# RobinChen121/Stochastic-Inventory

Measured on NVIDIA B200. Metric: state-action-demand evaluations/s (fp64), full-horizon SDP solve, higher is better.
Workload: dtype f64

## Files before the change

stochastic-inventory_b200/csrc/kernel_lead.cuh:

```cuda
#pragma once
#include <cuda_runtime.h>

#include <cstdlib>

#include "dev_model.cuh"
#include "kernel_tiled.cuh"

namespace sdpb {

constexpr int kLeadYT = 4;

struct LeadArgs {
    int t, D, pmf_off;
    const double* Vn;
    double* Vt;
    int* Qt;
    long long lo, hi;
    long long row0;
    int NYT;
    int ny_tiles, nq2_tiles;
    int A, Apad, di_max, NR;
    int nthreads;
};

__device__ __forceinline__ long long lds_s64(unsigned shared_addr) {
    long long v;
    asm volatile("ld.shared.s64 %0, [%1];" : "=l"(v) : "r"(shared_addr));
    return v;
}

__device__ __forceinline__ double ldg_at(const char* base, long long byte_off) {
    return __ldg(reinterpret_cast<const double*>(base + byte_off));
}

__device__ __forceinline__ double lds_double(unsigned shared_addr) {
    double v;
    asm volatile("ld.shared.f64 %0, [%1];" : "=d"(v) : "r"(shared_addr));
    return v;
}

template <bool IS_MIN, bool LAST, int RQ, bool DEDUP>
__global__ void __launch_bounds__(256)
bi_lead_slab(const __grid_constant__ DevModel M, const __grid_constant__ LeadArgs a) {
    constexpr int YT = kLeadYT;
    extern __shared__ __align__(16) unsigned char smem_raw[];
    const int NYB = YT * a.NYT;
    const int D = a.D, A = a.A, Apad = a.Apad;
    double* slab = reinterpret_cast<double*>(smem_raw);
    const size_t slab_elems = (size_t)max(a.NR, NYB) * RQ * Apad;
    double* Lw = slab + slab_elems;
    double2* PP = reinterpret_cast<double2*>(Lw + ((a.NR + 1) & ~1));

    long long b = blockIdx.x;
    int q2_0 = 0;
    if (M.lead == 2) { q2_0 = (int)(b % a.nq2_tiles) * RQ; b /= a.nq2_tiles; }
    const int ytile = (int)(b % a.ny_tiles); b /= a.ny_tiles;
    const long long ix = DEDUP ? 0 : a.row0 + b;
    const int q1_0 = ytile * NYB;
    const long long y0 = ix + q1_0;
    const int n_levels = DEDUP ? (M.nI + M.nQ - 1) : M.nQ;

    const int tid = threadIdx.x;
    for (int j = tid; j < D; j += a.nthreads) PP[j] = make_double2(M.pmf_p[a.pmf_off + j], M.pmf_pg[a.pmf_off + j]);
    const bool lost = (M.flags & SDPB_F_LOST_SALES) != 0;
    const long long strideX = (M.lead == 2) ? (long long)M.nQ * M.nQ : (long long)M.nQ;
    for (int wi = tid; wi < a.NR; wi += a.nthreads) {
        const double lvl = M.inv_min + (double)(y0 - a.di_max + wi) * M.step;
        Lw[wi] = M.h * fmax(lvl, 0.0) + M.pen * fmax(-lvl, 0.0);
    }
    if (!LAST) {
        const int warp_s = tid >> 5, lane_s = tid & 31, nwarps_s = a.nthreads >> 5;
        for (int row = warp_s; row < a.NR * RQ; row += nwarps_s) {
            const int wi = row / RQ, rr = row - wi * RQ;
            long long is = y0 - a.di_max + wi;
            if (lost) is = is > M.i_zero ? is : M.i_zero;
            is = is < M.nI - 1 ? is : M.nI - 1;
            is = is > 0 ? is : 0;
            const int q2 = min(q2_0 + rr, M.nQ - 1);
            const double* __restrict__ src = a.Vn + is * strideX + ((M.lead == 2) ? (long long)q2 * M.nQ : 0);
            const unsigned dst = (unsigned)__cvta_generic_to_shared(slab + (size_t)row * Apad);
            for (int ai = lane_s; ai < A; ai += 32)
                asm volatile("cp.async.ca.shared.global [%0], [%1], 8;" ::"r"(dst + (unsigned)ai * 8u), "l"(src + ai));
        }
        asm volatile("cp.async.commit_group;");
        asm volatile("cp.async.wait_group 0;" ::: "memory");
    }
    __syncthreads();

    const int g = tid / A, ai = tid - g * A;
    const bool worker = g < a.NYT;
    double acc[YT][RQ];
#pragma unroll
    for (int k = 0; k < YT; k++)
#pragma unroll
        for (int r = 0; r < RQ; r++) acc[k][r] = 0.0;

    if (worker) {
        const double av = (double)ai * M.step;
        const double fv = (av > 0.0 ? M.K : 0.0) + M.v_t[a.t - 1] * av;
        const unsigned slab_s = (unsigned)__cvta_generic_to_shared(slab) + (unsigned)ai * 8u;
        const unsigned lw_s = (unsigned)__cvta_generic_to_shared(Lw);
        const unsigned pp_s = (unsigned)__cvta_generic_to_shared(PP);
        const unsigned row_bytes = (unsigned)(RQ * Apad) * 8u;
        int wi0 = YT * g + (D - 1);
        double cst[YT], Vw[YT][RQ];
#pragma unroll
        for (int k = 0; k < YT; k++) {
            cst[k] = fv + lds_double(lw_s + (unsigned)(wi0 + k) * 8u);
#pragma unroll
            for (int r = 0; r < RQ; r++)
                Vw[k][r] = LAST ? 0.0 : lds_double(slab_s + (unsigned)(wi0 + k) * row_bytes + (unsigned)(r * Apad) * 8u);
        }
#define SDPB_LEAD_STEP(JJ)                                                                          \
        {                                                                                               \
            const double2 pp = lds_double2(pp_s + (unsigned)j * 16u);                                   \
            const int wn = max(wi0 - 1, 0);                                                             \
            const double lnew = lds_double(lw_s + (unsigned)wn * 8u);                                   \
            double vnew[RQ];                                                                            \
            _Pragma("unroll") for (int r = 0; r < RQ; r++)                                              \
                vnew[r] = LAST ? 0.0 : lds_double(slab_s + (unsigned)wn * row_bytes + (unsigned)(r * Apad) * 8u); \
            _Pragma("unroll") for (int k = 0; k < YT; k++) {                                            \
                const int ph = (k - (JJ)) & 3;                                                          \
                const double m = pp.x * cst[ph];                                \
                _Pragma("unroll") for (int r = 0; r < RQ; r++) {                                        \
                    acc[k][r] += m;                                     \
                    if (!LAST) acc[k][r] += pp.y * Vw[ph][r];           \
                }                                                                                       \
            }                                                                                           \
            const int pn = (3 - (JJ)) & 3;                                                              \
            cst[pn] = fv + lnew;                                                                        \
            _Pragma("unroll") for (int r = 0; r < RQ; r++) Vw[pn][r] = vnew[r];                         \
            wi0 -= 1;                                                                                   \
            j += 1;                                                                                     \
        }
        int j = 0;
        for (; j + 4 <= D;) { SDPB_LEAD_STEP(0) SDPB_LEAD_STEP(1) SDPB_LEAD_STEP(2) SDPB_LEAD_STEP(3) }
        if (j < D) SDPB_LEAD_STEP(0)
        if (j < D) SDPB_LEAD_STEP(1)
        if (j < D) SDPB_LEAD_STEP(2)
#undef SDPB_LEAD_STEP
    }

    __syncthreads();
    double* Qs = slab;
    if (worker) {
#pragma unroll
        for (int k = 0; k < YT; k++)
#pragma unroll
            for (int r = 0; r < RQ; r++) Qs[((size_t)(YT * g + k) * RQ + r) * Apad + ai] = acc[k][r];
    }
    __syncthreads();
    const int warp = tid >> 5, lane = tid & 31, nwarps = a.nthreads >> 5;
    for (int s = warp; s < NYB * RQ; s += nwarps) {
        const int local = s / RQ, r = s - local * RQ;
        const double* q = Qs + (size_t)s * Apad;
        double best = IS_MIN ? DBL_MAX : -DBL_MAX;
        int besti = kNoAction;
        for (int i = lane; i < A; i += 32) {
            const double v = q[i];
            if (IS_MIN ? (v < best) : (v > best)) { best = v; besti = i; }
        }
#pragma unroll
        for (int sh = 16; sh > 0; sh >>= 1) {
            const double ov = __shfl_xor_sync(0xffffffffu, best, sh);
            const int oi = __shfl_xor_sync(0xffffffffu, besti, sh);
            if (better<IS_MIN>(ov, oi, best, besti)) { best = ov; besti = oi; }
        }
        if (lane == 0) {
            const int lev = q1_0 + local;
            const int q2 = q2_0 + r;
            if (lev < n_levels && (M.lead != 2 || q2 < M.nQ)) {
                long long idx = DEDUP ? (long long)lev : ix * M.nQ + lev;
                if (M.lead == 2) idx = idx * M.nQ + q2;
                if (idx >= a.lo && idx < a.hi) {
                    a.Vt[idx] = best;
                    a.Qt[idx] = besti == kNoAction ? -1 : besti;
                }
            }
        }
    }
}

struct LeadPlan {
    bool ok = false;
    int NYT = 0, RQ = 1, Apad = 0, nthreads = 0, di_max = 0, span = 0, NR = 0;
// ... 147 lines not shown
            double pre = 0.0;
            if (!LAST) pre = ldg_at(col, lds_s64(ro_s + (unsigned)max(wi0 - 1, 0) * 8u));
#define SDPB_COL_STEP(JJ)                                                                             \
            {                                                                                             \
                const double2 pp = lds_double2(pp_s + (unsigned)j * 16u);                                 \
                const double vnew = pre;                                                                  \
                if (!LAST) pre = ldg_at(col, lds_s64(ro_s + (unsigned)max(wi0 - 2, 0) * 8u));             \
                const double lnew = lds_double(lw_s + (unsigned)max(wi0 - 1, 0) * 8u);                    \
                _Pragma("unroll") for (int k = 0; k < YT; k++) {                                          \
                    const int ph = (k - (JJ)) & (YT - 1);                                                 \
                    acc[k] += pp.x * cst[ph];                             \
                    if (!LAST) acc[k] += pp.y * Vw[ph];                   \
                }                                                                                         \
                const int pn = (YT - 1 - (JJ)) & (YT - 1);                                                \
                cst[pn] = fv + lnew;                                                                      \
                Vw[pn] = vnew;                                                                            \
                wi0 -= 1;                                                                                 \
                j += 1;                                                                                   \
            }
            int j = 0;
            for (; j + YT <= D;) {
#pragma unroll
                for (int jj = 0; jj < YT; jj++) SDPB_COL_STEP(jj)
            }
#pragma unroll
            for (int jj = 0; jj < YT - 1; jj++)
                if (j < D) SDPB_COL_STEP(jj)
#undef SDPB_COL_STEP
        }
#pragma unroll
        for (int k = 0; k < YT; k++) red_v[(size_t)k * a.nthreads + tid] = acc[k];
        __syncthreads();
        for (int s = warp; s < YT * a.NQB; s += nwarps) {
            const int k = s / a.NQB, sq = s - k * a.NQB;
            const double* q = red_v + (size_t)k * a.nthreads + sq * A;
            double best = IS_MIN ? DBL_MAX : -DBL_MAX;
            int besti = kNoAction;
            for (int i = lane; i < A; i += 32) {
                const double v = q[i];
                if (IS_MIN ? (v < best) : (v > best)) { best = v; besti = i; }
            }
#pragma unroll
            for (int sh = 16; sh > 0; sh >>= 1) {
                const double ov = __shfl_xor_sync(0xffffffffu, best, sh);
                const int oi = __shfl_xor_sync(0xffffffffu, besti, sh);
                if (better<IS_MIN>(ov, oi, best, besti)) { best = ov; besti = oi; }
            }
            if (lane == 0) {
                const int lev = l0 + k;
                const int sq2 = q2g * a.NQB + sq;
                if (lev < l_end && (M.lead != 2 || sq2 < M.nQ)) {
                    long long idx = DEDUP ? (long long)lev : ix * M.nQ + lev;
                    if (M.lead == 2) idx = idx * M.nQ + sq2;
                    if (idx >= a.lo && idx < a.hi) {
                        a.Vt[idx] = best;
                        a.Qt[idx] = besti == kNoAction ? -1 : besti;
                    }
                }
            }
        }
    }
}

struct ColPlan {
    bool ok = false;
    int NQB = 1, nthreads = 0, LT = 0, di_max = 0, span = 0, NRW = 0;
    size_t smem = 0;
};

inline ColPlan plan_col(const sdpb_model& m, const DevModel& d, int D, const int* di, bool dedup) {
    ColPlan P;
    if (m.cost_kind != SDPB_COST_BACKORDER || m.lead_time < 1) return P;
    int lo = di[0], hi = di[0];
    for (int j = 0; j < D; j++) {
        if (di[j] != di[0] + j) return P;
        lo = std::min(lo, di[j]);
        hi = std::max(hi, di[j]);
    }
    const int A = d.max_order_idx + 1;
    if (A > 512) return P;
    const int max_threads = 512;
    P.NQB = m.lead_time == 2 ? std::max(1, std::min(max_threads / A, d.nQ)) : 1;
    P.nthreads = ((P.NQB * A + 31) / 32) * 32;
    const int n_levels = dedup ? d.nI + d.nQ - 1 : d.nQ;
    P.LT = dedup ? 64 : ((n_levels + kColYT - 1) / kColYT) * kColYT;
    P.di_max = hi;
    P.span = hi - lo;
    P.NRW = P.LT + P.span;
    P.smem = ((((size_t)2 * kColYT * P.nthreads + 2 * (size_t)P.NRW) * 8 + 15) & ~(size_t)15) + (size_t)D * 16 + 16;
    P.ok = P.smem <= 100 * 1024;
    return P;
}

template <bool DEDUP>
inline int launch_col(const ColPlan& P, const DevModel& dm, int t, int D, int pmf_off, const double* Vn,
                      double* Vt, int* Qt, long long lo, long long hi, cudaStream_t stream) {
    if (hi <= lo) return SDPB_OK;
    ColArgs a;
    a.t = t; a.D = D; a.pmf_off = pmf_off; a.Vn = Vn; a.Vt = Vt; a.Qt = Qt; a.lo = lo; a.hi = hi;
    a.A = dm.max_order_idx + 1; a.NQB = P.NQB; a.LT = P.LT; a.di_max = P.di_max; a.NRW = P.NRW;
    a.nthreads = P.nthreads;
    a.nq2_groups = dm.lead == 2 ? (dm.nQ + P.NQB - 1) / P.NQB : 1;
    const int n_levels = DEDUP ? dm.nI + dm.nQ - 1 : dm.nQ;
    a.n_ltiles = (n_levels + P.LT - 1) / P.LT;
    long long rows = 1;
    a.row0 = 0;
    if (!DEDUP) {
        const long long per_x = dm.lead == 2 ? (long long)dm.nQ * dm.nQ : (long long)dm.nQ;
        a.row0 = lo / per_x;
        rows = (hi - 1) / per_x - a.row0 + 1;
    }
    const long long blocks = rows * a.n_ltiles * a.nq2_groups;
    const bool last = (Vn == nullptr), mn = dm.is_min != 0;
    cudaError_t e = cudaSuccess;
#define SDPB_COL_LAUNCH(MN, LS)                                                                        \
    {                                                                                                  \
        auto k = bi_lead_col<MN, LS, DEDUP>;                                                           \
        if (P.smem > 48 * 1024) e = cudaFuncSetAttribute(k, cudaFuncAttributeMaxDynamicSharedMemorySize, (int)P.smem); \
        if (e == cudaSuccess) k<<<(unsigned)blocks, P.nthreads, P.smem, stream>>>(dm, a);              \
    }
    if (mn) { if (last) SDPB_COL_LAUNCH(true, true) else SDPB_COL_LAUNCH(true, false) }
    else    { if (last) SDPB_COL_LAUNCH(false, true) else SDPB_COL_LAUNCH(false, false) }
#undef SDPB_COL_LAUNCH
    if (e != cudaSuccess || cudaGetLastError() != cudaSuccess) return SDPB_ERR_CUDA;
    return SDPB_OK;
}

struct DevPeer { char* base0; unsigned long long stride; long long lo, hi; };

template <bool IS_MIN>
__global__ void __launch_bounds__(256)
merge_action_slices(const double* __restrict__ sv, const int* __restrict__ sa, int parts, long long n_local,
                    double* __restrict__ Vt, int* __restrict__ Qt, long long lo, const DevPeer* __restrict__ peers,
                    int n_peers, int t) {
    const long long i = (long long)blockIdx.x * blockDim.x + threadIdx.x;
    if (i >= n_local) return;
    double best = IS_MIN ? DBL_MAX : -DBL_MAX;
    int arg = kNoAction;
    for (int q = 0; q < parts; q++) {
        const double v = sv[(long long)q * n_local + i];
        const int av = sa[(long long)q * n_local + i];
        if (av != kNoAction && (IS_MIN ? (v < best) : (v > best))) { best = v; arg = av; }
    }
    Vt[i] = best;
    Qt[i] = arg == kNoAction ? -1 : arg;
    const long long idx = lo + i;
    for (int p = 0; p < n_peers; p++) {
        const DevPeer pr = peers[p];
        if (idx >= pr.lo && idx < pr.hi)
            reinterpret_cast<double*>(pr.base0 + (unsigned long long)(t - 1) * pr.stride)[idx] = best;
    }
}

struct Q2Args {
    int t, D, pmf_off;
    const double* VnT;
    double* Vt;
    int* Qt;
    long long lo, hi;
    long long f_begin, f_end;
    int n_chunks, tpx;
    int cs;
    double* slice_v;
    int* slice_a;
    int di_max, NRW;
    int parts;
    int n_peer;
    double* peer_v[2];
    long long peer_lo[2], peer_hi[2];
};

struct PeerStore { double* v; long long lo, hi; };

constexpr int kQ2YT = 8, kQ2PF = 2, kQ2PAD = kQ2PF + 1;

__global__ void transpose_q2a(const double* __restrict__ V, double* __restrict__ VT, int nQ, int row0) {
    __shared__ double tile[32][33];
    const long long base = (long long)(row0 + blockIdx.x) * nQ * nQ;
    const int c0 = blockIdx.y * 32, r0 = blockIdx.z * 32;
    for (int r = threadIdx.y; r < 32; r += 8) {
        const int row = r0 + r, c = c0 + threadIdx.x;
        if (row < nQ && c < nQ) tile[r][threadIdx.x] = V[base + (long long)row * nQ + c];
    }
    __syncthreads();
    for (int r = threadIdx.y; r < 32; r += 8) {
        const int row = c0 + r, c = r0 + threadIdx.x;
        if (row < nQ && c < nQ) VT[base + (long long)row * nQ + c] = tile[threadIdx.x][r];
    }
}

template <bool IS_MIN, bool LAST, int NT, int PARTS>
__global__ void __launch_bounds__(NT, 512 / NT)
bi_lead_q2(const __grid_constant__ DevModel M, const __grid_constant__ Q2Args a) {
    constexpr int YT = kQ2YT, PF = kQ2PF, W = YT + PF, PAD = kQ2PAD;
    extern __shared__ __align__(16) unsigned char smem_raw[];
    double2* WR = reinterpret_cast<double2*>(smem_raw);
    double2* PP = WR + a.NRW;
    const int D = a.D, nQ = M.nQ, tid = threadIdx.x;
    constexpr int cols = NT / PARTS;
    const int part = tid / cols, col = tid - part * cols;
    double* MV = reinterpret_cast<double*>(PP + D);
    int* MA = reinterpret_cast<int*>(MV + (size_t)(PARTS - 1) * YT * cols);
    const long long F0 = a.f_begin + (long long)blockIdx.x * cols;
    const long long x_first = F0 / a.tpx;
    const bool lost = (M.flags & SDPB_F_LOST_SALES) != 0;

    for (int j = tid; j < D; j += NT) PP[j] = make_double2(M.pmf_p[a.pmf_off + j], M.pmf_pg[a.pmf_off + j]);
    for (int wi = tid; wi < a.NRW; wi += NT) {
        const long long il = x_first - a.di_max - PAD + wi;
        const double lvl = M.inv_min + (double)il * M.step;
        long long is = il;
        if (lost) is = is > M.i_zero ? is : M.i_zero;
        is = is < M.nI - 1 ? is : M.nI - 1;
        is = is > 0 ? is : 0;
        WR[wi] = make_double2(M.h * fmax(lvl, 0.0) + M.pen * fmax(-lvl, 0.0),
                              __hiloint2double(0, (int)(is * nQ * nQ)));
    }
    __syncthreads();

    const long long F = min(F0 + col, a.f_end - 1);
    const long long x = F / a.tpx;
    const int f = (int)(F - x * a.tpx);
    const int chunk = f / nQ, q2 = f - chunk * nQ, l0 = chunk * YT;
    const long long idx0 = (x * nQ + l0) * nQ + q2;
    bool any = false;
#pragma unroll
    for (int k = 0; k < YT; k++) any |= (l0 + k < nQ) && idx0 + (long long)k * nQ >= a.lo && idx0 + (long long)k * nQ < a.hi;
    any = any && F0 + col < a.f_end;
    if (PARTS == 1 && !any) return;

    const unsigned wr0 = (unsigned)__cvta_generic_to_shared(WR) + (unsigned)((int)(x - x_first) + l0 + (D - 1) + PAD) * 16u;
    const unsigned pp_s = (unsigned)__cvta_generic_to_shared(PP);
    const double* __restrict__ cb = LAST ? nullptr : a.VnT + q2;
    const double vt = M.v_t[a.t - 1];

    double best[YT];
    int arg[YT];
#pragma unroll
    for (int k = 0; k < YT; k++) { best[k] = IS_MIN ? DBL_MAX : -DBL_MAX; arg[k] = kNoAction; }

    const int per_part = (M.max_order_idx + PARTS) / PARTS;
    const int ai_begin = any ? part * per_part : 0;
    const int ai_end = any ? min(M.max_order_idx + 1, ai_begin + per_part) : 0;
    if (!LAST) cb += (long long)ai_begin * nQ;
    for (int ai = ai_begin; ai < ai_end; ai++) {
        const double av = (double)ai * M.step;
        const double fv = (av > 0.0 ? M.K : 0.0) + vt * av;
        double acc[YT], cst[W], Vw[W];
#pragma unroll
        for (int k = 0; k < YT; k++) acc[k] = 0.0;
#pragma unroll
        for (int k = 0; k < W; k++) {
            const double2 e = lds_double2(wr0 + (unsigned)((k < YT ? k : k - W) * 16));
            cst[k] = fv + e.x;
            Vw[k] = LAST ? 0.0 : __ldg(cb + __double2loint(e.y));
        }
        unsigned wr_run = wr0 - (unsigned)((PF + 1) * 16);
#define SDPB_Q2_STEP(JJ)                                                                              \
        {                                                                                                 \
            const double2 pp = lds_double2(pp_s + (unsigned)j * 16u);                                     \
            _Pragma("unroll") for (int k = 0; k < YT; k++) {                                              \
                acc[k] += pp.x * cst[(k - (JJ) + W) % W];                 \
                if (!LAST) acc[k] += pp.y * Vw[(k - (JJ) + W) % W];       \
            }                                                                                             \
            const double2 e = lds_double2(wr_run);             \
            cst[(YT - 1 - (JJ) + W) % W] = fv + e.x;                                                      \
            if (!LAST) Vw[(YT - 1 - (JJ) + W) % W] = __ldg(cb + __double2loint(e.y));                     \
            wr_run -= 16u;                                                                                \
            j += 1;                                                                                       \
        }
        int j = 0;
        while (j + W <= D) {
#pragma unroll
            for (int JJ = 0; JJ < W; JJ++) SDPB_Q2_STEP(JJ)
        }
#pragma unroll
        for (int JJ = 0; JJ < W - 1; JJ++)
            if (j < D) SDPB_Q2_STEP(JJ)
#undef SDPB_Q2_STEP
#pragma unroll
        for (int k = 0; k < YT; k++)
            if (IS_MIN ? (acc[k] < best[k]) : (acc[k] > best[k])) { best[k] = acc[k]; arg[k] = ai; }
        if (!LAST) cb += nQ;
    }
    if (PARTS > 1) {
        if (part > 0) {
#pragma unroll
            for (int k = 0; k < YT; k++) {
                MV[((part - 1) * YT + k) * cols + col] = best[k];
                MA[((part - 1) * YT + k) * cols + col] = arg[k];
            }
        }
        __syncthreads();
        if (part > 0 || !any) return;
        for (int q = 0; q < PARTS - 1; q++) {
#pragma unroll
            for (int k = 0; k < YT; k++) {
                const double v = MV[(q * YT + k) * cols + col];
                const int av = MA[(q * YT + k) * cols + col];
                if (av != kNoAction && (IS_MIN ? (v < best[k]) : (v > best[k]))) { best[k] = v; arg[k] = av; }
            }
        }
    }
#pragma unroll
    for (int k = 0; k < YT; k++) {
        const long long idx = idx0 + (long long)k * nQ;
        if (l0 + k < nQ && idx >= a.lo && idx < a.hi) {
            a.Vt[idx] = best[k];
            a.Qt[idx] = arg[k] == kNoAction ? -1 : arg[k];
            for (int p = 0; p < a.n_peer; p++)
                if (idx >= a.peer_lo[p] && idx < a.peer_hi[p]) a.peer_v[p][idx] = best[k];
        }
    }
}

template <int IMM>
__device__ __forceinline__ double2 lds_double2_o(unsigned shared_addr) {
    double2 v;
    asm volatile("ld.shared.v2.f64 {%0, %1}, [%2+%3];" : "=d"(v.x), "=d"(v.y) : "r"(shared_addr), "n"(IMM));
    return v;
}

constexpr int kQ2mNC = 3;
constexpr int kQ2mPW = kQ2YT;
constexpr unsigned short kQ2mNoAction = 0xffff;

struct Q2mLayout { int NG; unsigned off_rg, off_gb, off_pz, off_bv, off_ba, off_mt; size_t smem; };

__host__ __device__ inline Q2mLayout q2m_layout(int NRW, int D, int NT, int cs) {
    Q2mLayout L;
    L.NG = (NT - 1) / cs + 2;
    const unsigned R = (unsigned)(D + kQ2YT - 1);
    unsigned o = (unsigned)(NRW + D) * 16u;
    L.off_rg = o; o += (unsigned)L.NG * R * 16u;
    L.off_gb = o; o += ((unsigned)L.NG * 4u + 15u) & ~15u;
    L.off_pz = o; o += ((R + kQ2YT - 1) * 8u + 15u) & ~15u;
    L.off_bv = o; o += (unsigned)(kQ2mNC * kQ2YT * NT) * 8u;
    L.off_ba = o; o += ((unsigned)(kQ2mNC * kQ2YT * NT) * 2u + 15u) & ~15u;
    L.off_mt = o; o += (unsigned)L.NG * R * 64u;
    L.smem = o;
    return L;
}

template <bool LAST, int KLO, int KHI, int PH, int VS, int IMM>
__device__ __forceinline__ void q2m_diag(double (&acc)[kQ2mNC][kQ2YT], unsigned mt, const double (&pw)[kQ2mPW],
                                         const double (&vb)[kQ2mNC][2]) {
    double mm[kQ2YT];
    if (KLO < 2 && KHI > 0) { const double2 t = lds_double2_o<IMM>(mt); mm[0] = t.x; mm[1] = t.y; }
    if (KLO < 4 && KHI > 2) { const double2 t = lds_double2_o<IMM + 16>(mt); mm[2] = t.x; mm[3] = t.y; }
    if (KLO < 6 && KHI > 4) { const double2 t = lds_double2_o<IMM + 32>(mt); mm[4] = t.x; mm[5] = t.y; }
    if (KLO < 8 && KHI > 6) { const double2 t = lds_double2_o<IMM + 48>(mt); mm[6] = t.x; mm[7] = t.y; }
#pragma unroll
    for (int k = KLO; k < KHI; k++)
#pragma unroll
        for (int c = 0; c < kQ2mNC; c++) {
            acc[c][k] += mm[k];
            if (!LAST) acc[c][k] += pw[(PH + k) % kQ2mPW] * vb[c][VS];
        }
}

template <int VS, int PS, int IMM>
__device__ __forceinline__ void q2m_refill(double (&pw)[kQ2mPW], double (&vb)[kQ2mNC][2], unsigned rg,
                                           const double* const (&cb)[kQ2mNC]) {
    const double2 r = lds_double2_o<IMM>(rg);
    if (PS >= 0) pw[PS < 0 ? 0 : PS] = r.x;
    const unsigned off = (unsigned)__double2loint(r.y);
#pragma unroll
    for (int c = 0; c < kQ2mNC; c++) vb[c][VS] = __ldg(cb[c] + off);
}

template <bool IS_MIN, bool LAST, int NT>
__global__ void __launch_bounds__(NT, 512 / NT)
bi_lead_q2m(const __grid_constant__ DevModel M, const __grid_constant__ Q2Args a) {
    constexpr int YT = kQ2YT, PAD = kQ2PAD, NC = kQ2mNC, PW = kQ2mPW;
    static_assert(YT == 8 && NC == 3 && PW == 8, "the diagonals below are written out for these sizes");
    static_assert(NT % 8 == 0, "the table builder keeps the slot index fixed per thread");
    extern __shared__ __align__(16) unsigned char smem_raw[];
    const int D = a.D, nQ = M.nQ, cs = a.cs, tid = threadIdx.x;
    const int R = D + YT - 1;
    const Q2mLayout L = q2m_layout(a.NRW, D, NT, cs);
    double2* WR = reinterpret_cast<double2*>(smem_raw);
    double2* PP = WR + a.NRW;
    double2* RG = reinterpret_cast<double2*>(smem_raw + L.off_rg);
    int* GB = reinterpret_cast<int*>(smem_raw + L.off_gb);
    double* PZ = reinterpret_cast<double*>(smem_raw + L.off_pz);
    double* BV = reinterpret_cast<double*>(smem_raw + L.off_bv);
    unsigned short* BA = reinterpret_cast<unsigned short*>(smem_raw + L.off_ba);
    double* MT = reinterpret_cast<double*>(smem_raw + L.off_mt);
    const int NG = L.NG;
    const long long F0 = a.f_begin + (long long)blockIdx.x * NT;
    const long long x_first = F0 / a.tpx;
    const long long G0 = F0 / cs;
    const bool lost = (M.flags & SDPB_F_LOST_SALES) != 0;

    for (int j = tid; j < D; j += NT) PP[j] = make_double2(M.pmf_p[a.pmf_off + j], M.pmf_pg[a.pmf_off + j]);
    for (int j = tid; j < R + YT - 1; j += NT) {
        const int jd = j - (YT - 1);
        PZ[j] = jd >= 0 && jd < D ? M.pmf_p[a.pmf_off + jd] : 0.0;
    }
    for (int wi = tid; wi < a.NRW; wi += NT) {
        const long long il = x_first - a.di_max - PAD + wi;
        const double lvl = M.inv_min + (double)il * M.step;
        long long is = il;
        if (lost) is = is > M.i_zero ? is : M.i_zero;
        is = is < M.nI - 1 ? is : M.nI - 1;
        is = is > 0 ? is : 0;
        WR[wi] = make_double2(M.h * fmax(lvl, 0.0) + M.pen * fmax(-lvl, 0.0),
                              __hiloint2double(0, (int)(is * nQ * nQ)));
    }
    for (int g = tid; g < NG; g += NT) {
        const long long G = G0 + g;
        const long long xg = G / a.n_chunks;
        const int chunk = (int)(G - xg * a.n_chunks);
        int wb = (int)(xg - x_first) + chunk * YT + (D - 1) + PAD;
        GB[g] = min(wb, a.NRW - YT);
    }
#pragma unroll
    for (int s2 = 0; s2 < NC * YT; s2++) { BV[s2 * NT + tid] = IS_MIN ? DBL_MAX : -DBL_MAX; BA[s2 * NT + tid] = kQ2mNoAction; }
    __syncthreads();
    for (int e = tid; e < NG * R; e += NT) {
        const int g = e / R, n = e - g * R;
        RG[e] = make_double2(n + 1 < D ? PP[n + 1].y : 0.0, WR[GB[g] + 5 - n].y);
    }

    const long long F = min(F0 + tid, a.f_end - 1);
    const long long x = F / a.tpx;
    const int f = (int)(F - x * a.tpx);
    const int chunk = f / cs, c0 = f - chunk * cs, l0 = chunk * YT;
    const int g_own = (int)(F / cs - G0);
    const long long idx0 = (x * nQ + l0) * nQ + c0;
    const long long idx_end = idx0 + (long long)(min(YT, nQ - l0) - 1) * nQ + (long long)((nQ - 1 - c0) / cs) * cs;
    const bool any = F0 + tid < a.f_end && idx_end >= a.lo && idx0 < a.hi;

    const unsigned wr_s = (unsigned)__cvta_generic_to_shared(WR);
    const unsigned pp_s = (unsigned)__cvta_generic_to_shared(PP);
    const unsigned rg0 = (unsigned)__cvta_generic_to_shared(RG) + (unsigned)(g_own * R) * 16u;
    const unsigned mt0 = (unsigned)__cvta_generic_to_shared(MT) + (unsigned)(g_own * R) * 64u;
    const unsigned bv_s = (unsigned)__cvta_generic_to_shared(BV) + (unsigned)tid * 8u;
    const unsigned ba_s = (unsigned)__cvta_generic_to_shared(BA) + (unsigned)tid * 2u;
    const int gb = (int)(x - x_first) + l0 + (D - 1) + PAD;
    const double* cb[NC];
#pragma unroll
    for (int c = 0; c < NC; c++) cb[c] = LAST ? nullptr : a.VnT + c0 + (c0 + c * cs < nQ ? c * cs : 0);
    const double vt = M.v_t[a.t - 1];

    const int n_sl = (int)gridDim.y, sl = (int)blockIdx.y;
    const int per_sl = (M.max_order_idx + n_sl) / n_sl;
    const int ai_begin = sl * per_sl, ai_end = min(M.max_order_idx + 1, ai_begin + per_sl);
#pragma unroll
    for (int c = 0; c < NC; c++) if (!LAST) cb[c] += (long long)ai_begin * nQ;
    for (int ai = ai_begin; ai < ai_end; ai++) {
        {
            const double av = (double)ai * M.step;
            const double fv = (av > 0.0 ? M.K : 0.0) + vt * av;
            for (int r = tid; r < NG * R; r += NT) {
                const int g = r / R, n = r - g * R;
                const double cst = fv + WR[GB[g] + (YT - 1) - n].x;
                double2* Mr = reinterpret_cast<double2*>(MT + (size_t)r * YT);
#pragma unroll
                for (int k = 0; k < YT; k += 2)
                    Mr[k / 2] = make_double2(PZ[n + k] * cst, PZ[n + k + 1] * cst);
            }
        }
        __syncthreads();
        if (any) {
            double acc[NC][YT];
#pragma unroll
            for (int c = 0; c < NC; c++)
#pragma unroll
                for (int k = 0; k < YT; k++) acc[c][k] = 0.0;
            if (D >= YT - 1) {
                double pw[PW], vb[NC][2];
                if (!LAST) {
                    pw[0] = lds_double(pp_s + 8u);
#pragma unroll
                    for (int n = 0; n < 2; n++) {
                        const unsigned off = (unsigned)__double2loint(lds_double(wr_s + (unsigned)(gb + 7 - n) * 16u + 8u));
#pragma unroll
                        for (int c = 0; c < NC; c++) vb[c][n] = __ldg(cb[c] + off);
                    }
                }
#define SDPB_Q2M_HEAD(N)                                                                              \
                q2m_diag<LAST, YT - 1 - (N), YT, (N) + 1, (N) & 1, (N) * 64>(acc, mt0, pw, vb);           \
                if (!LAST) q2m_refill<(N) & 1, (N) + 1, (N) * 16>(pw, vb, rg0, cb);
                SDPB_Q2M_HEAD(0) SDPB_Q2M_HEAD(1) SDPB_Q2M_HEAD(2) SDPB_Q2M_HEAD(3)
                SDPB_Q2M_HEAD(4) SDPB_Q2M_HEAD(5) SDPB_Q2M_HEAD(6)
#undef SDPB_Q2M_HEAD
#define SDPB_Q2M_FULL(U)                                                                              \
                q2m_diag<LAST, 0, YT, (U), ((U) + 1) & 1, (U) * 64>(acc, mt_run, pw, vb);                 \
                if (!LAST) q2m_refill<((U) + 1) & 1, (U), (U) * 16>(pw, vb, rg_run, cb);
                int n = YT - 1;
                unsigned mt_run = mt0 + (unsigned)n * 64u, rg_run = rg0 + (unsigned)n * 16u;
                for (; n + PW <= D; n += PW, mt_run += PW * 64u, rg_run += PW * 16u) {
                    SDPB_Q2M_FULL(0) SDPB_Q2M_FULL(1) SDPB_Q2M_FULL(2) SDPB_Q2M_FULL(3) SDPB_Q2M_FULL(4)
                    SDPB_Q2M_FULL(5) SDPB_Q2M_FULL(6) SDPB_Q2M_FULL(7)
                }
                if (n + 0 < D) { SDPB_Q2M_FULL(0) }
                if (n + 1 < D) { SDPB_Q2M_FULL(1) }
                if (n + 2 < D) { SDPB_Q2M_FULL(2) }
                if (n + 3 < D) { SDPB_Q2M_FULL(3) }
                if (n + 4 < D) { SDPB_Q2M_FULL(4) }
                if (n + 5 < D) { SDPB_Q2M_FULL(5) }
                if (n + 6 < D) { SDPB_Q2M_FULL(6) }
                if (n + 7 < D) { SDPB_Q2M_FULL(7) }
#undef SDPB_Q2M_FULL
                double pe[PW], ve[NC][2];
                if (!LAST) {
#pragma unroll
                    for (int m = 0; m < YT - 1; m++) pe[m] = lds_double(pp_s + (unsigned)(D - (YT - 1) + m) * 16u + 8u);
                    const bool odd = (D & 1) != 0;
#pragma unroll
                    for (int c = 0; c < NC; c++) {
                        ve[c][0] = odd ? vb[c][1] : vb[c][0];
                        ve[c][1] = odd ? vb[c][0] : vb[c][1];
                    }
                }
                const unsigned mt_d = mt0 + (unsigned)D * 64u, rg_d = rg0 + (unsigned)D * 16u;
#define SDPB_Q2M_TAIL(E)                                                                              \
                q2m_diag<LAST, 0, YT - 1 - (E), (E), (E) & 1, (E) * 64>(acc, mt_d, pe, ve);               \
                if (!LAST && (E) + 2 < YT - 1) q2m_refill<(E) & 1, -1, (E) * 16>(pe, ve, rg_d, cb);
                SDPB_Q2M_TAIL(0) SDPB_Q2M_TAIL(1) SDPB_Q2M_TAIL(2) SDPB_Q2M_TAIL(3)
                SDPB_Q2M_TAIL(4) SDPB_Q2M_TAIL(5) SDPB_Q2M_TAIL(6)
#undef SDPB_Q2M_TAIL
            } else {
                for (int n = 0; n < R; n++) {
                    double mm[YT], v[NC];
                    if (!LAST) {
                        const unsigned off = (unsigned)__double2loint(lds_double(wr_s + (unsigned)(gb + 7 - n) * 16u + 8u));
#pragma unroll
                        for (int c = 0; c < NC; c++) v[c] = __ldg(cb[c] + off);
                    }
#pragma unroll
                    for (int p = 0; p < YT / 2; p++) {
                        const double2 t = lds_double2(mt0 + (unsigned)n * 64u + (unsigned)p * 16u);
                        mm[2 * p] = t.x; mm[2 * p + 1] = t.y;
                    }
#pragma unroll
                    for (int k = 0; k < YT; k++) {
                        const int j = n - (YT - 1) + k;
                        if (j < 0 || j >= D) continue;
                        const double pg = LAST ? 0.0 : lds_double(pp_s + (unsigned)j * 16u + 8u);
#pragma unroll
                        for (int c = 0; c < NC; c++) {
                            acc[c][k] += mm[k];
                            if (!LAST) acc[c][k] += pg * v[c];
                        }
                    }
                }
            }
#pragma unroll
            for (int c = 0; c < NC; c++)
#pragma unroll
                for (int k = 0; k < YT; k++) {
                    const unsigned so = (unsigned)((c * YT + k) * NT);
                    const double bv = lds_double(bv_s + so * 8u);
                    if (IS_MIN ? (acc[c][k] < bv) : (acc[c][k] > bv)) {
                        asm volatile("st.shared.f64 [%0], %1;" ::"r"(bv_s + so * 8u), "d"(acc[c][k]) : "memory");
                        asm volatile("st.shared.u16 [%0], %1;" ::"r"(ba_s + so * 2u), "h"((unsigned short)ai) : "memory");
                    }
                }
        }
        __syncthreads();
#pragma unroll
        for (int c = 0; c < NC; c++) if (!LAST) cb[c] += nQ;
    }
    if (!any) return;
    unsigned ts;
    asm volatile("mov.u32 %0, %%tid.x;" : "=r"(ts));
    const long long Fs = min(F0 + (long long)ts, a.f_end - 1);
    const long long xs = Fs / a.tpx;
    const int fs = (int)(Fs - xs * a.tpx);
    const int cks = fs / cs, c0s = fs - cks * cs, l0s = cks * YT;
    const long long idx0s = (xs * nQ + l0s) * nQ + c0s;
#pragma unroll
    for (int c = 0; c < NC; c++) {
        if (c0s + c * cs >= nQ) break;
#pragma unroll
        for (int k = 0; k < YT; k++) {
            const long long idx = idx0s + (long long)k * nQ + c * cs;
            if (!(l0s + k < nQ && idx >= a.lo && idx < a.hi)) continue;
            const double best = BV[(c * YT + k) * NT + ts];
            const unsigned short ba = BA[(c * YT + k) * NT + ts];
            const int arg = ba == kQ2mNoAction ? kNoAction : (int)ba;
            if (n_sl > 1) {
                a.slice_v[(long long)sl * (a.hi - a.lo) + (idx - a.lo)] = best;
                a.slice_a[(long long)sl * (a.hi - a.lo) + (idx - a.lo)] = arg;
                continue;
            }
            a.Vt[idx] = best;
            a.Qt[idx] = arg == kNoAction ? -1 : arg;
            for (int p = 0; p < a.n_peer; p++)
                if (idx >= a.peer_lo[p] && idx < a.peer_hi[p]) a.peer_v[p][idx] = best;
        }
    }
}

struct Q2Plan {
    bool ok = false;
    int NT = 128, n_chunks = 0, tpx = 0, di_max = 0, NRW = 0;
    size_t smem = 0;
};

inline Q2Plan plan_q2(const sdpb_model& m, const DevModel& d, int D, const int* di) {
    Q2Plan P;
    if (m.cost_kind != SDPB_COST_BACKORDER || m.lead_time != 2) return P;
    for (int j = 0; j < D; j++)
        if (di[j] != di[0] + j) return P;
    if ((long long)d.nI * d.nQ * d.nQ >= 0x7fffffffLL) return P;
    P.n_chunks = (d.nQ + kQ2YT - 1) / kQ2YT;
    P.tpx = P.n_chunks * d.nQ;
    P.di_max = di[D - 1];
    const int dx_max = (P.NT + P.tpx - 1) / P.tpx + 1;
    P.NRW = P.n_chunks * kQ2YT + D + kQ2PAD + dx_max;
    P.smem = (size_t)(P.NRW + D) * 16 + (size_t)kQ2YT * P.NT * 12;
    P.ok = P.smem <= 96 * 1024;
    return P;
}

constexpr int kQ2MaxPeers = 2;

struct Q2Shape { bool shared; int parts, slices, cs, tpx, NRW; long long f_begin, f_end; Q2mLayout L; };

inline Q2Shape q2_shape(const Q2Plan& P, const DevModel& dm, int D, long long lo, long long hi, int sm_count) {
    Q2Shape S{};
    const long long per_x = (long long)dm.nQ * dm.nQ;
    const long long rows = (hi - 1) / per_x - lo / per_x + 1;
    const double waves = (double)(rows * P.tpx) / 32.0 / (16.0 * sm_count);
    S.parts = waves >= 6.0 ? 1 : (waves >= 3.0 ? 2 : 4);
    S.cs = (dm.nQ + kQ2mNC - 1) / kQ2mNC;
    const int tpx2 = P.n_chunks * S.cs;
    const int NRW2 = P.n_chunks * kQ2YT + D + kQ2PAD + (P.NT + tpx2 - 1) / tpx2 + 1;
    S.slices = 1;
    S.L = q2m_layout(NRW2, D, P.NT, S.cs);
    static const bool force_share = std::getenv("SDPB_Q2_SHARE") != nullptr;
    static const int force_split = [] { const char* e = std::getenv("SDPB_Q2_SPLIT"); return e ? std::atoi(e) : 0; }();
    if (force_split) {
        S.parts = force_split == 2 ? 2 : 4;
    } else if (S.L.smem <= 56 * 1024) {
        S.shared = true; S.parts = 1;
        const double ctas = (double)(rows * tpx2) / P.NT;
        const double w = ctas / (4.0 * sm_count);
        if (w < 8.0 && !force_share) S.slices = (int)std::min(8.0, std::ceil(8.0 / std::max(w, 0.01)));
        S.slices = std::max(1, std::min(S.slices, (dm.max_order_idx + 1) / 8));
        const int per = (dm.max_order_idx + S.slices) / S.slices;
        S.slices = (dm.max_order_idx + per) / per;
    }
    S.tpx = S.shared ? tpx2 : P.tpx;
    S.NRW = S.shared ? NRW2 : P.NRW;
    S.f_begin = (lo / per_x) * S.tpx;
    S.f_end = ((hi - 1) / per_x + 1) * S.tpx;
    return S;
}

inline int launch_q2(const Q2Plan& P, const Q2Shape& S, const DevModel& dm, int t, int D, int pmf_off, const double* Vn,
                     double* VnT, double* Vt, int* Qt, long long lo, long long hi, int row0, int row1, cudaStream_t stream,
                     const PeerStore* peers, int n_peers, double* slice_v, int* slice_a, size_t slice_cap,
                     const DevPeer* d_peers, int n_dev_peers) {
    if (hi <= lo) return SDPB_OK;
    const bool last = (Vn == nullptr), mn = dm.is_min != 0;
    if (!last) {
        const unsigned tiles = (unsigned)((dm.nQ + 31) / 32);
        transpose_q2a<<<dim3((unsigned)(row1 - row0), tiles, tiles), dim3(32, 8), 0, stream>>>(Vn, VnT, dm.nQ, row0);
    }
    const long long n_local = hi - lo;
    if (S.slices > 1 && (size_t)S.slices * (size_t)n_local > slice_cap) return SDPB_ERR_NOMEM;
    Q2Args a;
    a.t = t; a.D = D; a.pmf_off = pmf_off; a.VnT = last ? nullptr : VnT; a.Vt = Vt; a.Qt = Qt; a.lo = lo; a.hi = hi;
    a.n_chunks = P.n_chunks; a.tpx = S.tpx; a.di_max = P.di_max; a.NRW = S.NRW;
    a.f_begin = S.f_begin; a.f_end = S.f_end; a.parts = S.parts; a.cs = S.cs;
    a.slice_v = slice_v; a.slice_a = slice_a;
    a.n_peer = 0;
    for (int p = 0; p < kQ2MaxPeers; p++) { a.peer_v[p] = nullptr; a.peer_lo[p] = a.peer_hi[p] = 0; }
    if (S.slices == 1)
        for (int p = 0; p < n_peers && p < kQ2MaxPeers; p++) {
            a.peer_v[p] = peers[p].v; a.peer_lo[p] = peers[p].lo; a.peer_hi[p] = peers[p].hi;
            a.n_peer = p + 1;
        }
    const int cols = P.NT / a.parts;
    const Q2mLayout L = S.L;
    const bool shared = S.shared;
    cudaError_t e = cudaSuccess;
    const dim3 grid((unsigned)((a.f_end - a.f_begin + cols - 1) / cols), (unsigned)S.slices);
#define SDPB_Q2_LAUNCH(K, SMEM, GRID)                                                                  \
    {                                                                                                  \
        auto k = K;                                                                                    \
        if (SMEM > 48 * 1024) e = cudaFuncSetAttribute(k, cudaFuncAttributeMaxDynamicSharedMemorySize, (int)SMEM); \
        if (e == cudaSuccess) k<<<GRID, 128, SMEM, stream>>>(dm, a);                                   \
    }
#define SDPB_Q2_NT(MN, LS)                                                                             \
    if (shared) SDPB_Q2_LAUNCH((bi_lead_q2m<MN, LS, 128>), L.smem, grid)                               \
    else if (a.parts == 1) SDPB_Q2_LAUNCH((bi_lead_q2<MN, LS, 128, 1>), P.smem, grid.x)                \
    else if (a.parts == 2) SDPB_Q2_LAUNCH((bi_lead_q2<MN, LS, 128, 2>), P.smem, grid.x)                \
    else SDPB_Q2_LAUNCH((bi_lead_q2<MN, LS, 128, 4>), P.smem, grid.x)
    if (mn) { if (last) SDPB_Q2_NT(true, true) else SDPB_Q2_NT(true, false) }
    else    { if (last) SDPB_Q2_NT(false, true) else SDPB_Q2_NT(false, false) }
#undef SDPB_Q2_NT
#undef SDPB_Q2_LAUNCH
    if (e != cudaSuccess || cudaGetLastError() != cudaSuccess) return SDPB_ERR_CUDA;
    if (S.slices > 1) {
        const unsigned mb = (unsigned)((n_local + 255) / 256);
        if (mn) merge_action_slices<true><<<mb, 256, 0, stream>>>(slice_v, slice_a, S.slices, n_local, Vt + lo, Qt + lo, lo, d_peers, n_dev_peers, t);
        else merge_action_slices<false><<<mb, 256, 0, stream>>>(slice_v, slice_a, S.slices, n_local, Vt + lo, Qt + lo, lo, d_peers, n_dev_peers, t);
        if (cudaGetLastError() != cudaSuccess) return SDPB_ERR_CUDA;
    }
    return SDPB_OK;
}

}
```

Before: 4436 billion.

## Double-buffer per-action cost tables and remap q2m tiles along the first lead axis

Tiles in the shared q2m kernel now group 8 consecutive x levels with q1 fixed, instead of 8 consecutive q1 values. The grid is re-indexed from a row0 base to match. The per-action cost matrix is double-buffered when shared memory allows, so building the next action's table overlaps the current evaluation and one __syncthreads per action is removed. Precomputed packed row offsets and a shifted pmf copy reduce index arithmetic in the table build. This uses more shared memory, which may reduce occupancy, and rewrites output indexing, which carries a correctness risk.

After: 4622 billion, median of 6. +4.2%, better.

```diff
diff --git a/stochastic-inventory_b200/csrc/kernel_lead.cuh b/stochastic-inventory_b200/csrc/kernel_lead.cuh
--- a/stochastic-inventory_b200/csrc/kernel_lead.cuh
+++ b/stochastic-inventory_b200/csrc/kernel_lead.cuh
@@ -31,6 +31,12 @@
 
 __device__ __forceinline__ double ldg_at(const char* base, long long byte_off) {
     return __ldg(reinterpret_cast<const double*>(base + byte_off));
+}
+
+__device__ __forceinline__ unsigned lds_u32(unsigned shared_addr) {
+    unsigned v;
+    asm volatile("ld.shared.u32 %0, [%1];" : "=r"(v) : "r"(shared_addr));
+    return v;
 }
 
 __device__ __forceinline__ double lds_double(unsigned shared_addr) {
@@ -484,6 +490,8 @@
     }
 }
 
+struct Q2mLayout { int NG, nbuf; unsigned off_rg, off_gb, off_br, off_pz, off_bv, off_ba, off_mt; size_t smem; };
+
 struct Q2Args {
     int t, D, pmf_off;
     const double* VnT;
@@ -493,6 +501,7 @@
     long long f_begin, f_end;
     int n_chunks, tpx;
     int cs;
+    long long row0;
     double* slice_v;
     int* slice_a;
     int di_max, NRW;
@@ -657,20 +666,24 @@
 constexpr int kQ2mPW = kQ2YT;
 constexpr unsigned short kQ2mNoAction = 0xffff;
 
-struct Q2mLayout { int NG; unsigned off_rg, off_gb, off_pz, off_bv, off_ba, off_mt; size_t smem; };
+constexpr size_t kQ2mSmemMax = 56 * 1024;
 
 __host__ __device__ inline Q2mLayout q2m_layout(int NRW, int D, int NT, int cs) {
     Q2mLayout L;
     L.NG = (NT - 1) / cs + 2;
     const unsigned R = (unsigned)(D + kQ2YT - 1);
     unsigned o = (unsigned)(NRW + D) * 16u;
-    L.off_rg = o; o += (unsigned)L.NG * R * 16u;
+    L.off_rg = o; o += (unsigned)L.NG * (R + 2) * 16u;
     L.off_gb = o; o += ((unsigned)L.NG * 4u + 15u) & ~15u;
-    L.off_pz = o; o += ((R + kQ2YT - 1) * 8u + 15u) & ~15u;
+    L.off_br = o; o += ((unsigned)L.NG * R * 4u + 15u) & ~15u;
+    const unsigned pz = ((R + kQ2YT - 1) * 8u + 15u) & ~15u;
+    L.off_pz = o; o += 2u * pz;
     L.off_bv = o; o += (unsigned)(kQ2mNC * kQ2YT * NT) * 8u;
     L.off_ba = o; o += ((unsigned)(kQ2mNC * kQ2YT * NT) * 2u + 15u) & ~15u;
-    L.off_mt = o; o += (unsigned)L.NG * R * 64u;
-    L.smem = o;
+    L.off_mt = o;
+    const size_t mt = (size_t)L.NG * R * 64u;
+    L.nbuf = o + 2 * mt <= kQ2mSmemMax ? 2 : 1;
+    L.smem = o + L.nbuf * mt;
     return L;
 }
 
@@ -699,6 +712,16 @@
     const unsigned off = (unsigned)__double2loint(r.y);
 #pragma unroll
     for (int c = 0; c < kQ2mNC; c++) vb[c][VS] = __ldg(cb[c] + off);
+}
+
+__device__ __forceinline__ void q2m_build_row(unsigned cost, unsigned prow, unsigned dst, double fv) {
+    const double cst = fv + lds_double(cost);
+#pragma unroll
+    for (int p = 0; p < kQ2YT / 2; p++) {
+        const double2 z = lds_double2(prow + (unsigned)p * 16u);
+        asm volatile("st.shared.v2.f64 [%0], {%1, %2};" ::"r"(dst + (unsigned)p * 16u), "d"(z.x * cst), "d"(z.y * cst)
+                     : "memory");
+    }
 }
 
 template <bool IS_MIN, bool LAST, int NT>
@@ -715,20 +738,24 @@
     double2* PP = WR + a.NRW;
     double2* RG = reinterpret_cast<double2*>(smem_raw + L.off_rg);
     int* GB = reinterpret_cast<int*>(smem_raw + L.off_gb);
-    double* PZ = reinterpret_cast<double*>(smem_raw + L.off_pz);
+    unsigned* BR = reinterpret_cast<unsigned*>(smem_raw + L.off_br);
+    const unsigned pz_bytes = ((unsigned)(R + YT - 1) * 8u + 15u) & ~15u;
+    double* PZ0 = reinterpret_cast<double*>(smem_raw + L.off_pz);
+    double* PZ1 = reinterpret_cast<double*>(smem_raw + L.off_pz + pz_bytes);
     double* BV = reinterpret_cast<double*>(smem_raw + L.off_bv);
     unsigned short* BA = reinterpret_cast<unsigned short*>(smem_raw + L.off_ba);
-    double* MT = reinterpret_cast<double*>(smem_raw + L.off_mt);
     const int NG = L.NG;
     const long long F0 = a.f_begin + (long long)blockIdx.x * NT;
-    const long long x_first = F0 / a.tpx;
+    const long long X_first = F0 / a.tpx;
+    const long long x_first = a.row0 + X_first * YT;
     const long long G0 = F0 / cs;
     const bool lost = (M.flags & SDPB_F_LOST_SALES) != 0;
 
     for (int j = tid; j < D; j += NT) PP[j] = make_double2(M.pmf_p[a.pmf_off + j], M.pmf_pg[a.pmf_off + j]);
     for (int j = tid; j < R + YT - 1; j += NT) {
         const int jd = j - (YT - 1);
-        PZ[j] = jd >= 0 && jd < D ? M.pmf_p[a.pmf_off + jd] : 0.0;
+        PZ0[j] = jd >= 0 && jd < D ? M.pmf_p[a.pmf_off + jd] : 0.0;
+        PZ1[j] = jd + 1 >= 0 && jd + 1 < D ? M.pmf_p[a.pmf_off + jd + 1] : 0.0;
     }
     for (int wi = tid; wi < a.NRW; wi += NT) {
         const long long il = x_first - a.di_max - PAD + wi;
@@ -742,60 +769,65 @@
     }
     for (int g = tid; g < NG; g += NT) {
         const long long G = G0 + g;
-        const long long xg = G / a.n_chunks;
-        const int chunk = (int)(G - xg * a.n_chunks);
-        int wb = (int)(xg - x_first) + chunk * YT + (D - 1) + PAD;
+        const long long Xg = G / nQ;
+        const int q1g = (int)(G - Xg * nQ);
+        int wb = (int)(Xg - X_first) * YT + q1g + (D - 1) + PAD;
         GB[g] = min(wb, a.NRW - YT);
     }
 #pragma unroll
     for (int s2 = 0; s2 < NC * YT; s2++) { BV[s2 * NT + tid] = IS_MIN ? DBL_MAX : -DBL_MAX; BA[s2 * NT + tid] = kQ2mNoAction; }
     __syncthreads();
-    for (int e = tid; e < NG * R; e += NT) {
+    const int NGR = NG * R;
+    for (int e = tid; e < NGR; e += NT) {
         const int g = e / R, n = e - g * R;
-        RG[e] = make_double2(n + 1 < D ? PP[n + 1].y : 0.0, WR[GB[g] + 5 - n].y);
-    }
+        RG[g * (R + 2) + n + 2] = make_double2(n + 1 < D ? PP[n + 1].y : 0.0, WR[GB[g] + 5 - n].y);
+        if (n < 2) RG[g * (R + 2) + n] = make_double2(n == 1 ? PP[0].y : 0.0, WR[GB[g] + 7 - n].y);
+        const unsigned pz = L.off_pz + ((n & 1) ? pz_bytes + (unsigned)(n - 1) * 8u : (unsigned)n * 8u);
+        BR[e] = (unsigned)(reinterpret_cast<unsigned char*>(&WR[GB[g] + (YT - 1) - n]) - smem_raw) << 16 | pz;
+    }
+
+    const unsigned sm_s = (unsigned)__cvta_generic_to_shared(smem_raw);
+    const unsigned br_s = sm_s + L.off_br;
+    const unsigned mt_base = sm_s + L.off_mt;
+    const unsigned mt_buf = (unsigned)NGR * 64u;
+    const bool dbl = L.nbuf == 2;
+    const double vt = M.v_t[a.t - 1];
+    const auto build = [&](int ab, unsigned mt) {
+        const double av = (double)ab * M.step;
+        const double fv = (av > 0.0 ? M.K : 0.0) + vt * av;
+        for (int r = tid; r < NGR; r += NT) {
+            const unsigned br = lds_u32(br_s + (unsigned)r * 4u);
+            q2m_build_row(sm_s + (br >> 16), sm_s + (br & 0xffffu), mt + (unsigned)r * 64u, fv);
+        }
+    };
 
     const long long F = min(F0 + tid, a.f_end - 1);
-    const long long x = F / a.tpx;
-    const int f = (int)(F - x * a.tpx);
-    const int chunk = f / cs, c0 = f - chunk * cs, l0 = chunk * YT;
+    const long long X = F / a.tpx;
+    const int f = (int)(F - X * a.tpx);
+    const int q1 = f / cs, c0 = f - q1 * cs;
     const int g_own = (int)(F / cs - G0);
-    const long long idx0 = (x * nQ + l0) * nQ + c0;
-    const long long idx_end = idx0 + (long long)(min(YT, nQ - l0) - 1) * nQ + (long long)((nQ - 1 - c0) / cs) * cs;
+    const long long idx0 = ((a.row0 + X * YT) * nQ + q1) * nQ + c0;
+    const long long idx_end = idx0 + (long long)(YT - 1) * nQ * nQ + (long long)((nQ - 1 - c0) / cs) * cs;
     const bool any = F0 + tid < a.f_end && idx_end >= a.lo && idx0 < a.hi;
 
-    const unsigned wr_s = (unsigned)__cvta_generic_to_shared(WR);
     const unsigned pp_s = (unsigned)__cvta_generic_to_shared(PP);
-    const unsigned rg0 = (unsigned)__cvta_generic_to_shared(RG) + (unsigned)(g_own * R) * 16u;
-    const unsigned mt0 = (unsigned)__cvta_generic_to_shared(MT) + (unsigned)(g_own * R) * 64u;
-    const unsigned bv_s = (unsigned)__cvta_generic_to_shared(BV) + (unsigned)tid * 8u;
-    const unsigned ba_s = (unsigned)__cvta_generic_to_shared(BA) + (unsigned)tid * 2u;
-    const int gb = (int)(x - x_first) + l0 + (D - 1) + PAD;
+    const unsigned rg0 = (unsigned)__cvta_generic_to_shared(RG) + (unsigned)(g_own * (R + 2) + 2) * 16u;
     const double* cb[NC];
 #pragma unroll
     for (int c = 0; c < NC; c++) cb[c] = LAST ? nullptr : a.VnT + c0 + (c0 + c * cs < nQ ? c * cs : 0);
-    const double vt = M.v_t[a.t - 1];
 
     const int n_sl = (int)gridDim.y, sl = (int)blockIdx.y;
     const int per_sl = (M.max_order_idx + n_sl) / n_sl;
     const int ai_begin = sl * per_sl, ai_end = min(M.max_order_idx + 1, ai_begin + per_sl);
 #pragma unroll
     for (int c = 0; c < NC; c++) if (!LAST) cb[c] += (long long)ai_begin * nQ;
+    if (dbl) build(ai_begin, mt_base);
     for (int ai = ai_begin; ai < ai_end; ai++) {
-        {
-            const double av = (double)ai * M.step;
-            const double fv = (av > 0.0 ? M.K : 0.0) + vt * av;
-            for (int r = tid; r < NG * R; r += NT) {
-                const int g = r / R, n = r - g * R;
-                const double cst = fv + WR[GB[g] + (YT - 1) - n].x;
-                double2* Mr = reinterpret_cast<double2*>(MT + (size_t)r * YT);
-#pragma unroll
-                for (int k = 0; k < YT; k += 2)
-                    Mr[k / 2] = make_double2(PZ[n + k] * cst, PZ[n + k + 1] * cst);
-            }
-        }
+        if (!dbl) build(ai, mt_base);
         __syncthreads();
+        if (dbl && ai + 1 < ai_end) build(ai + 1, mt_base + (unsigned)((ai + 1 - ai_begin) & 1) * mt_buf);
         if (any) {
+            const unsigned mt0 = mt_base + (dbl ? (unsigned)((ai - ai_begin) & 1) * mt_buf : 0u) + (unsigned)(g_own * R) * 64u;
             double acc[NC][YT];
 #pragma unroll
             for (int c = 0; c < NC; c++)
@@ -807,7 +839,7 @@
                     pw[0] = lds_double(pp_s + 8u);
 #pragma unroll
                     for (int n = 0; n < 2; n++) {
-                        const unsigned off = (unsigned)__double2loint(lds_double(wr_s + (unsigned)(gb + 7 - n) * 16u + 8u));
+                        const unsigned off = (unsigned)__double2loint(lds_double(rg0 + (unsigned)(n - 2) * 16u + 8u));
 #pragma unroll
                         for (int c = 0; c < NC; c++) vb[c][n] = __ldg(cb[c] + off);
                     }
@@ -858,7 +890,7 @@
                 for (int n = 0; n < R; n++) {
                     double mm[YT], v[NC];
                     if (!LAST) {
-                        const unsigned off = (unsigned)__double2loint(lds_double(wr_s + (unsigned)(gb + 7 - n) * 16u + 8u));
+                        const unsigned off = (unsigned)__double2loint(lds_double(rg0 + (unsigned)(n - 2) * 16u + 8u));
 #pragma unroll
                         for (int c = 0; c < NC; c++) v[c] = __ldg(cb[c] + off);
                     }
@@ -880,6 +912,9 @@
                     }
                 }
             }
+            unsigned tr;
+            asm volatile("mov.u32 %0, %%tid.x;" : "=r"(tr));
+            const unsigned bv_s = sm_s + L.off_bv + tr * 8u, ba_s = sm_s + L.off_ba + tr * 2u;
 #pragma unroll
             for (int c = 0; c < NC; c++)
 #pragma unroll
@@ -892,7 +927,7 @@
                     }
                 }
         }
-        __syncthreads();
+        if (!dbl) __syncthreads();
 #pragma unroll
         for (int c = 0; c < NC; c++) if (!LAST) cb[c] += nQ;
     }
@@ -900,17 +935,17 @@
     unsigned ts;
     asm volatile("mov.u32 %0, %%tid.x;" : "=r"(ts));
     const long long Fs = min(F0 + (long long)ts, a.f_end - 1);
-    const long long xs = Fs / a.tpx;
-    const int fs = (int)(Fs - xs * a.tpx);
-    const int cks = fs / cs, c0s = fs - cks * cs, l0s = cks * YT;
-    const long long idx0s = (xs * nQ + l0s) * nQ + c0s;
+    const long long Xs = Fs / a.tpx;
+    const int fs = (int)(Fs - Xs * a.tpx);
+    const int q1s = fs / cs, c0s = fs - q1s * cs;
+    const long long idx0s = ((a.row0 + Xs * YT) * nQ + q1s) * nQ + c0s;
 #pragma unroll
     for (int c = 0; c < NC; c++) {
         if (c0s + c * cs >= nQ) break;
 #pragma unroll
         for (int k = 0; k < YT; k++) {
-            const long long idx = idx0s + (long long)k * nQ + c * cs;
-            if (!(l0s + k < nQ && idx >= a.lo && idx < a.hi)) continue;
+            const long long idx = idx0s + (long long)k * nQ * nQ + c * cs;
+            if (!(idx >= a.lo && idx < a.hi)) continue;
             const double best = BV[(c * YT + k) * NT + ts];
             const unsigned short ba = BA[(c * YT + k) * NT + ts];
             const int arg = ba == kQ2mNoAction ? kNoAction : (int)ba;
@@ -951,7 +986,7 @@
 
 constexpr int kQ2MaxPeers = 2;
 
-struct Q2Shape { bool shared; int parts, slices, cs, tpx, NRW; long long f_begin, f_end; Q2mLayout L; };
+struct Q2Shape { bool shared; int parts, slices, cs, tpx, NRW; long long f_begin, f_end, row0; Q2mLayout L; };
 
 inline Q2Shape q2_shape(const Q2Plan& P, const DevModel& dm, int D, long long lo, long long hi, int sm_count) {
     Q2Shape S{};
@@ -960,17 +995,19 @@
     const double waves = (double)(rows * P.tpx) / 32.0 / (16.0 * sm_count);
     S.parts = waves >= 6.0 ? 1 : (waves >= 3.0 ? 2 : 4);
     S.cs = (dm.nQ + kQ2mNC - 1) / kQ2mNC;
-    const int tpx2 = P.n_chunks * S.cs;
-    const int NRW2 = P.n_chunks * kQ2YT + D + kQ2PAD + (P.NT + tpx2 - 1) / tpx2 + 1;
+    const int tpx2 = dm.nQ * S.cs;
+    const int dX = (P.NT + tpx2 - 1) / tpx2;
+    const int NRW2 = kQ2YT * dX + dm.nQ + kQ2YT - 1 + D + kQ2PAD;
+    const long long xchunks = (rows + kQ2YT - 1) / kQ2YT;
     S.slices = 1;
     S.L = q2m_layout(NRW2, D, P.NT, S.cs);
     static const bool force_share = std::getenv("SDPB_Q2_SHARE") != nullptr;
     static const int force_split = [] { const char* e = std::getenv("SDPB_Q2_SPLIT"); return e ? std::atoi(e) : 0; }();
     if (force_split) {
         S.parts = force_split == 2 ? 2 : 4;
-    } else if (S.L.smem <= 56 * 1024) {
+    } else if (S.L.smem <= kQ2mSmemMax) {
         S.shared = true; S.parts = 1;
-        const double ctas = (double)(rows * tpx2) / P.NT;
+        const double ctas = (double)(xchunks * tpx2) / P.NT;
         const double w = ctas / (4.0 * sm_count);
         if (w < 8.0 && !force_share) S.slices = (int)std::min(8.0, std::ceil(8.0 / std::max(w, 0.01)));
         S.slices = std::max(1, std::min(S.slices, (dm.max_order_idx + 1) / 8));
@@ -979,8 +1016,9 @@
     }
     S.tpx = S.shared ? tpx2 : P.tpx;
     S.NRW = S.shared ? NRW2 : P.NRW;
-    S.f_begin = (lo / per_x) * S.tpx;
-    S.f_end = ((hi - 1) / per_x + 1) * S.tpx;
+    S.row0 = lo / per_x;
+    S.f_begin = S.shared ? 0 : (lo / per_x) * S.tpx;
+    S.f_end = S.shared ? xchunks * S.tpx : ((hi - 1) / per_x + 1) * S.tpx;
     return S;
 }
 
@@ -999,7 +1037,7 @@
     Q2Args a;
     a.t = t; a.D = D; a.pmf_off = pmf_off; a.VnT = last ? nullptr : VnT; a.Vt = Vt; a.Qt = Qt; a.lo = lo; a.hi = hi;
     a.n_chunks = P.n_chunks; a.tpx = S.tpx; a.di_max = P.di_max; a.NRW = S.NRW;
-    a.f_begin = S.f_begin; a.f_end = S.f_end; a.parts = S.parts; a.cs = S.cs;
+    a.f_begin = S.f_begin; a.f_end = S.f_end; a.row0 = S.row0; a.parts = S.parts; a.cs = S.cs;
     a.slice_v = slice_v; a.slice_a = slice_a;
     a.n_peer = 0;
     for (int p = 0; p < kQ2MaxPeers; p++) { a.peer_v[p] = nullptr; a.peer_lo[p] = a.peer_hi[p] = 0; }
```
